# vsu/foo-dsp-bfir

Measured on AMD Instinct MI355X. Metric: Msamples/s (output channel-samples), 8ch 131072-tap FIR @4096-sample partitions, higher is better.
Workload: dtype f32; 1 GPU; cfg3_8ch_131072tap_L4096_fp32; channels=8, taps=131072, partition=4096, fft_size=8192, partitions=32, blocks_per_launch=4096, engines_rank0=1, channels_rank0=8, streams_total=1, io=interleaved frames resident in HBM (generated there), parallelism=one independent stream per rank, no collective

## Files before the change

foo-dsp-bfir_amd/csrc/fft_lds.h:

```cpp
#pragma once
#include <hip/hip_runtime.h>

#include <type_traits>

namespace bfir {

template <typename T, int P> __device__ __forceinline__ void pin_registers(T (&re)[P], T (&im)[P])
{
#pragma unroll
    for (int e = 0; e < P; e++) asm volatile("" : "+v"(re[e]), "+v"(im[e]));
}

template <typename T> struct Vec2;
template <> struct Vec2<float>  { using type = float2; };
template <> struct Vec2<double> { using type = double2; };
template <typename T> struct Vec4;
template <> struct Vec4<float>  { using type = float4; };
template <> struct Vec4<double> { using type = double4; };

template <int LOG2M> struct FftCfg;
#define BFIR_FFT_CFG(lg, nt, np, a, b, c, d)                                   \
    template <> struct FftCfg<lg> {                                            \
        static constexpr int NT = nt, NP = np, R0 = a, R1 = b, R2 = c, R3 = d; \
    };
BFIR_FFT_CFG(4, 4, 2, 4, 4, 1, 1)
BFIR_FFT_CFG(5, 4, 2, 8, 4, 1, 1)
BFIR_FFT_CFG(6, 8, 2, 8, 8, 1, 1)
BFIR_FFT_CFG(7, 16, 3, 8, 4, 4, 1)
BFIR_FFT_CFG(8, 16, 2, 16, 16, 1, 1)
BFIR_FFT_CFG(9, 32, 3, 16, 8, 4, 1)
BFIR_FFT_CFG(10, 64, 3, 16, 16, 4, 1)
BFIR_FFT_CFG(11, 128, 3, 16, 16, 8, 1)
BFIR_FFT_CFG(12, 256, 3, 16, 16, 16, 1)
BFIR_FFT_CFG(13, 512, 4, 16, 16, 8, 4)
BFIR_FFT_CFG(14, 1024, 4, 16, 16, 16, 4)
#undef BFIR_FFT_CFG

constexpr int BFIR_MIN_LOG2M = 4;
constexpr int BFIR_MAX_LOG2M = 14;

template <typename T>
__device__ __forceinline__ void cmul(T &re, T &im, T wr, T wi)
{
    T tr = re * wr - im * wi;
    T ti = re * wi + im * wr;
    re = tr; im = ti;
}

template <int MM, int SIGN, typename T>
__device__ __forceinline__ void mul_w16(T &re, T &im)
{
// ... 91 lines not shown

template <int LO, int HI, typename Fn> __device__ __forceinline__ void static_for(Fn &&f)
{
    if constexpr (LO < HI) {
        f(std::integral_constant<int, LO>{});
        static_for<LO + 1, HI>(f);
    }
}

__host__ __device__ constexpr int tw_nbase(int R) { return R == 16 ? 6 : R == 8 ? 4 : R == 4 ? 2 : 1; }
__host__ __device__ constexpr int tw_base_exp(int R, int j)
{
    return R == 16 ? (j < 4 ? j + 1 : 4 * (j - 2)) : j + 1;
}

template <typename T, int LOG2M, int SIGN> struct LdsFft {
    using Cfg = FftCfg<LOG2M>;
    using V2 = typename Vec2<T>::type;
    static constexpr int M = 1 << LOG2M;
    static constexpr int NT = Cfg::NT;
    static constexpr int P = M / NT;
    static constexpr int NP = Cfg::NP;

    __host__ __device__ static constexpr int radix(int s)
    {
        return s == 0 ? Cfg::R0 : s == 1 ? Cfg::R1 : s == 2 ? Cfg::R2 : Cfg::R3;
    }
    __host__ __device__ static constexpr int pprod(int s)
    {
        int p = 1;
        for (int j = 0; j < s; j++) p *= radix(j);
        return p;
    }
    __host__ __device__ static constexpr int twoff(int s)
    {
        int o = 0;
        for (int j = 1; j < s; j++) o += (radix(j) - 1) * pprod(j);
        return o;
    }
    __host__ __device__ static constexpr int twsize() { return twoff(NP); }

    static constexpr int LDS_ELEMS = M + M / 32;
    __host__ __device__ __forceinline__ static constexpr int phys(int i) { return i + (i >> 5); }

    __host__ __device__ __forceinline__ static constexpr int in_index(int tid, int e)
    {
        return (tid + (e / radix(0)) * NT) + (e % radix(0)) * (M / radix(0));
    }
    __host__ __device__ __forceinline__ static constexpr int out_index(int tid, int e)
    {
        return (tid + (e / radix(NP - 1)) * NT) + Dft<radix(NP - 1), SIGN, T>::inv(e % radix(NP - 1)) * (M / radix(NP - 1));
    }

    template <int S> static constexpr int ntw() { return S == 0 ? 1 : (P / radix(S)) * (radix(S) - 1); }

    template <int S>
    __device__ __forceinline__ static void load_twiddles(V2 (&w)[ntw<S>()], const V2 *__restrict__ tw, int tid)
    {
        constexpr int R = radix(S), p = pprod(S);
#pragma unroll
        for (int b = 0; b < P / R; b++) {
            const int k = (tid + b * NT) & (p - 1);
#pragma unroll
            for (int r = 1; r < R; r++) w[b * (R - 1) + r - 1] = tw[twoff(S) + (r - 1) * p + k];
        }
    }
// ... 25 lines not shown
        } else {
            exchange<S - 1>(re, im, lds, tid);
            load_twiddles<S>(w, tw, tid);
        }
        butterflies<S>(re, im, w);
    }

    template <int S> __host__ __device__ static constexpr int widx(int tid, int b, int q)
    {
        const int R = radix(S), p = pprod(S);
        const int i = tid + b * NT, k = i & (p - 1);
        return (i - k) * R + k + q * p;
    }
    template <int S> __host__ __device__ static constexpr int ridx(int tid, int b, int r)
    {
        return (tid + b * NT) + r * (M / radix(S + 1));
    }
    template <int S> __host__ __device__ static constexpr bool wr_affine()
    {
        for (int b = 0; b < P / radix(S); b++)
            for (int q = 0; q < radix(S); q++) {
                const int off = phys(widx<S>(0, b, q)) - phys(widx<S>(0, 0, 0));
                for (int t = 1; t < NT; t++)
                    if (phys(widx<S>(t, b, q)) - phys(widx<S>(t, 0, 0)) != off) return false;
            }
        return true;
    }
    template <int S> __host__ __device__ static constexpr bool rd_affine()
    {
        for (int b = 0; b < P / radix(S + 1); b++)
            for (int r = 0; r < radix(S + 1); r++) {
                const int off = phys(ridx<S>(0, b, r)) - phys(ridx<S>(0, 0, 0));
                for (int t = 1; t < NT; t++)
                    if (phys(ridx<S>(t, b, r)) - phys(ridx<S>(t, 0, 0)) != off) return false;
            }
        return true;
    }

    template <int S>
    __device__ __forceinline__ static void exchange(T *re, T *im, V2 *lds, int tid)
    {
        constexpr int R = radix(S), Rn = radix(S + 1);
        __syncthreads();
        if constexpr (wr_affine<S>()) {
            V2 *wp = lds + phys(widx<S>(tid, 0, 0));
            static_for<0, P / R>([&](auto B_) {
                constexpr int b = decltype(B_)::value;
                static_for<0, R>([&](auto Q_) {
                    constexpr int q = decltype(Q_)::value;
                    constexpr int off = phys(widx<S>(0, b, q)) - phys(widx<S>(0, 0, 0));
                    V2 v; v.x = re[b * R + Dft<R, SIGN, T>::pos(q)]; v.y = im[b * R + Dft<R, SIGN, T>::pos(q)];
                    wp[off] = v;
                });
            });
        } else {
#pragma unroll
            for (int b = 0; b < P / R; b++)
#pragma unroll
                for (int q = 0; q < R; q++) {
                    V2 v; v.x = re[b * R + Dft<R, SIGN, T>::pos(q)]; v.y = im[b * R + Dft<R, SIGN, T>::pos(q)];
                    lds[phys(widx<S>(tid, b, q))] = v;
                }
        }
        __syncthreads();
        if constexpr (rd_affine<S>()) {
            const V2 *rp = lds + phys(ridx<S>(tid, 0, 0));
            static_for<0, P / Rn>([&](auto B_) {
                constexpr int b = decltype(B_)::value;
                static_for<0, Rn>([&](auto R_) {
                    constexpr int r = decltype(R_)::value;
                    constexpr int off = phys(ridx<S>(0, b, r)) - phys(ridx<S>(0, 0, 0));
                    const V2 v = rp[off];
                    re[b * Rn + r] = v.x; im[b * Rn + r] = v.y;
                });
            });
        } else {
#pragma unroll
            for (int b = 0; b < P / Rn; b++)
#pragma unroll
                for (int r = 0; r < Rn; r++) {
                    V2 v = lds[phys(ridx<S>(tid, b, r))];
                    re[b * Rn + r] = v.x; im[b * Rn + r] = v.y;
                }
        }
#pragma unroll
        for (int e = 0; e < P; e++) asm volatile("" : "+v"(re[e]), "+v"(im[e]));
    }

    __host__ __device__ static constexpr int kspan(int s) { return pprod(s) < NT ? pprod(s) : NT; }
    __host__ __device__ static constexpr int boff(int s)
    {
        int o = 0;
        for (int j = 1; j < s; j++) o += tw_nbase(radix(j)) * kspan(j);
        return o;
    }
    __host__ __device__ static constexpr int bsize() { return boff(NP); }
    static constexpr int NBREG = NP > 1 ? tw_nbase(radix(NP - 1)) : 1;
    static constexpr int LDSB_ELEMS = NP > 2 ? boff(NP - 1) : 1;

    __device__ __forceinline__ static void load_bases(V2 (&B)[NBREG], V2 *ldsb, const V2 *__restrict__ twb, int tid)
    {
        if constexpr (NP > 2)
            for (int i = tid; i < LDSB_ELEMS; i += NT) ldsb[i] = twb[i];
        if constexpr (NP > 1)
            static_for<0, NBREG>([&](auto J_) {
                constexpr int J = decltype(J_)::value;
                B[J] = twb[boff(NP - 1) + J * kspan(NP - 1) + (tid & (kspan(NP - 1) - 1))];
            });
    }

    template <int S, int J> __device__ __forceinline__ static V2 base(const V2 (&B)[NBREG], const V2 *ldsb, int tid)
    {
        if constexpr (S == NP - 1) return B[J];
        else return ldsb[boff(S) + J * kspan(S) + (tid & (kspan(S) - 1))];
    }

    template <int S, int r> __device__ __forceinline__ static V2 base_twiddle(const V2 (&B)[NBREG], const V2 *ldsb, int tid)
    {
        constexpr int R = radix(S);
        if constexpr (R == 16 && (r & 3) != 0 && (r >> 2) != 0) {
            const V2 a = base<S, 2 + (r >> 2)>(B, ldsb, tid), c = base<S, (r & 3) - 1>(B, ldsb, tid);
            V2 w; w.x = a.x * c.x - a.y * c.y; w.y = a.x * c.y + a.y * c.x;
            return w;
        } else if constexpr (R == 16) {
            return base<S, ((r >> 2) == 0 ? r - 1 : 2 + (r >> 2))>(B, ldsb, tid);
        } else if constexpr (R == 8 && r > 4) {
            const V2 a = base<S, 3>(B, ldsb, tid), c = base<S, r - 5>(B, ldsb, tid);
            V2 w; w.x = a.x * c.x - a.y * c.y; w.y = a.x * c.y + a.y * c.x;
            return w;
        } else if constexpr (R == 4 && r == 3) {
            const V2 a = base<S, 0>(B, ldsb, tid), c = base<S, 1>(B, ldsb, tid);
            V2 w; w.x = a.x * c.x - a.y * c.y; w.y = a.x * c.y + a.y * c.x;
            return w;
        } else {
            return base<S, r - 1>(B, ldsb, tid);
        }
    }

    template <int S>
    __device__ __forceinline__ static void butterflies_tb(T *re, T *im, const V2 (&B)[NBREG], const V2 *ldsb, int tid)
    {
        constexpr int R = radix(S), p = pprod(S);
        static_assert(p <= NT || 16 * NT == p * R, "constant rotations are sixteenth roots of unity");
        static_for<1, R>([&](auto R_) {
            constexpr int r = decltype(R_)::value;
            if constexpr (R == 16 && (r & 3) == 0) __builtin_amdgcn_sched_barrier(0);
            const V2 w = base_twiddle<S, r>(B, ldsb, tid);
            static_for<0, P / R>([&](auto B_) {
                constexpr int b = decltype(B_)::value;
                constexpr int bp = b % (p > NT ? p / NT : 1);
                cmul(re[b * R + r], im[b * R + r], w.x, (T)(SIGN < 0 ? w.y : -w.y));
                if constexpr (bp != 0) mul_w16<(r * bp) % 16, SIGN>(re[b * R + r], im[b * R + r]);
            });
        });
        static_for<0, P / R>([&](auto B_) {
            constexpr int b = decltype(B_)::value;
            Dft<R, SIGN, T>::run(re + b * R, im + b * R);
        });
    }

    __device__ __forceinline__ static void run(T *re, T *im, V2 *lds, const V2 *__restrict__ tw, int tid)
    {
        {
            V2 w0[1];
            butterflies<0>(re, im, w0);
        }
        if constexpr (NP > 1) pass<1>(re, im, lds, tw, tid);
        if constexpr (NP > 2) pass<2>(re, im, lds, tw, tid);
        if constexpr (NP > 3) pass<3>(re, im, lds, tw, tid);
    }
};

}
```

foo-dsp-bfir_amd/csrc/kernels.hip:

```cpp
#include "kernels.h"

#include <algorithm>
#include <cmath>
#include <cstdio>
#include <cstdlib>
#include <vector>

#include "fft_lds.h"

namespace bfir {

constexpr int BFIR_MAXCH = 8;

#define BFIR_FOR_LOG2M(F) \
    F(4) F(5) F(6) F(7) F(8) F(9) F(10) F(11) F(12) F(13) F(14)

template <int LOG2M> static void fill_tw(std::vector<long double> &tw)
{
    using F = LdsFft<float, LOG2M, -1>;
    tw.assign(2 * (size_t)(F::twsize() > 0 ? F::twsize() : 1), 0.0L);
    const long double two_pi = 6.283185307179586476925286766559L;
    for (int s = 1; s < F::NP; s++) {
        const int R = F::radix(s), p = F::pprod(s);
        for (int r = 1; r < R; r++)
            for (int k = 0; k < p; k++) {
                long double ang = -two_pi * (long double)(r * k) / (long double)(p * R);
                size_t o = (size_t)F::twoff(s) + (size_t)(r - 1) * p + k;
                tw[2 * o] = cosl(ang);
                tw[2 * o + 1] = sinl(ang);
            }
    }
}

template <int LOG2M> static void fill_twb(std::vector<long double> &tw)
{
    using F = LdsFft<float, LOG2M, -1>;
    tw.assign(2 * (size_t)(F::bsize() > 0 ? F::bsize() : 1), 0.0L);
    const long double two_pi = 6.283185307179586476925286766559L;
    for (int s = 1; s < F::NP; s++) {
        const int R = F::radix(s), p = F::pprod(s), ks = F::kspan(s);
        for (int j = 0; j < tw_nbase(R); j++)
            for (int k0 = 0; k0 < ks; k0++) {
                long double ang = -two_pi * (long double)(tw_base_exp(R, j) * k0) / (long double)(p * R);
                size_t o = (size_t)F::boff(s) + (size_t)j * ks + k0;
                tw[2 * o] = cosl(ang);
                tw[2 * o + 1] = sinl(ang);
            }
    }
}

template <typename T> static void *upload(const std::vector<long double> &v)
{
    std::vector<T> h(v.size());
    for (size_t i = 0; i < v.size(); i++) h[i] = (T)v[i];
    void *d = nullptr;
    if (hipMalloc(&d, h.size() * sizeof(T)) != hipSuccess) return nullptr;
    if (hipMemcpy(d, h.data(), h.size() * sizeof(T), hipMemcpyHostToDevice) != hipSuccess) {
        (void)hipFree(d);
        return nullptr;
    }
    return d;
}

// ... 4 lines not shown
        BFIR_FOR_LOG2M(F)
#undef F
    }
    return 0;
}

int fft_plan_create(FftPlan *plan, int filter_length, int realsize)
{
    int lg = 0;
    while ((1 << lg) < filter_length) lg++;
    if ((1 << lg) != filter_length || lg < BFIR_MIN_LOG2M || lg > BFIR_MAX_LOG2M) return -1;
    if (realsize != 4 && realsize != 8) return -1;
    if (((size_t)filter_length + (size_t)filter_length / 32) * 2 * (size_t)realsize > 160 * 1024) return -1;
    std::vector<long double> tw, ws, twb;
    switch (lg) {
#define F(lgv) case lgv: fill_tw<lgv>(tw); fill_twb<lgv>(twb); break;
        BFIR_FOR_LOG2M(F)
#undef F
    }
    const int M = filter_length, N = 2 * M;
    ws.resize(2 * (size_t)M);
    const long double two_pi = 6.283185307179586476925286766559L;
    for (int k = 0; k < M; k++) {
        long double ang = -two_pi * (long double)k / (long double)N;
        ws[2 * k] = cosl(ang);
        ws[2 * k + 1] = sinl(ang);
    }
    plan->log2m = lg;
    plan->realsize = realsize;
    plan->tw = realsize == 4 ? upload<float>(tw) : upload<double>(tw);
    plan->ws = realsize == 4 ? upload<float>(ws) : upload<double>(ws);
// ... 2012 lines not shown
```

foo-dsp-bfir_amd/csrc/pair.hip:

```cpp
#include "kernels.h"

#include <algorithm>
#include <cstdlib>

#include "fft_lds.h"
#include "pair_io.h"

namespace bfir {

namespace {

template <int LOG2N>
__global__ __launch_bounds__(FftCfg<LOG2N>::NT, 4) void k_fwd_pair_ps(FwdPairArgs a, const float2 *__restrict__ twb, int run_len)
{
    using F = LdsFft<float, LOG2N, -1>;
    constexpr int N = F::M, NT = F::NT, P = F::P, L = N / 2, H = P / 2;
    static_assert(F::radix(0) == 16 && P == 16, "in_index(tid, e) = tid + e * (N / 16)");
    static_assert(F::phys(32) == 33 && F::phys(N - 1) == N - 1 + N / 32 - 1, "the split step's addresses assume i + (i >> 5)");
    __shared__ __attribute__((aligned(16))) float2 lds[F::LDS_ELEMS + 1];
    __shared__ __attribute__((aligned(16))) float2 ldsb[F::LDSB_ELEMS];

    const int tid = threadIdx.x;
    const int w = xcd_work_item(blockIdx.x, gridDim.x);
    const int half_c = a.C / 2, pairs = a.n_eng * half_c;
    const int rr = w / pairs, pp = w - rr * pairs;
    const float sc = 0.5f * a.scale;
    const int g = pp / half_c, cp = pp - g * half_c;
    const int C = a.C;
    const int t0 = rr * run_len, t1 = min(a.n_t, t0 + run_len);
    if (t0 >= t1) return;
// ... 48 lines not shown
            F::template butterflies<0>(re, im, w0);
        }
        static_for<1, F::NP>([&](auto S_) {
            constexpr int S = decltype(S_)::value;
            int tl = tid; asm volatile("" : "+v"(tl));
            F::template exchange<S - 1>(re, im, lds, tl);
            F::template butterflies_tb<S>(re, im, B, ldsb, tl);
            if constexpr (S == 1) {
                asm_prefetch8x2(nxt, fo, make_rsrc_words(raw + (long)(t + 1) * L * C, t + 1 < t1 ? blk_bytes : 0u), estep);
            }
        });

        int tz = tid; asm volatile("" : "+v"(tz));
        __syncthreads();
        {
            float2 *zw = lds + F::phys(tz);
            static_for<0, P>([&](auto E_) {
                constexpr int e = decltype(E_)::value;
                static_assert(F::out_index(0, e) % 32 == 0, "additive padding");
                float2 v; v.x = re[e]; v.y = im[e];
                zw[F::phys(F::out_index(0, e))] = v;
            });
        }
        __syncthreads();
        const long slot = (long)((a.base_slot + t) % a.ring) * N;
        const __amdgpu_buffer_rsrc_t rxa = make_rsrc(da0 + slot, (unsigned)N * 4u), rxb = make_rsrc(da0 + a.dst_ch_stride + slot, (unsigned)N * 4u);
        const float2 *zk = lds + F::phys(2 * tz);
        constexpr int OMAX = F::phys(2 * NT * (P / 4 - 1));
        const float2 *zn1 = lds + (F::phys(N - 1 - 2 * tz) - OMAX);
        const float2 *zn0 = zn1 + ((tz & 15) == 0 ? 2 : 1);
#pragma unroll
// ... 11 lines not shown
                const float2 zh = lds[F::phys(L)];
                const bool k0 = tz == 0;
                xa.x = k0 ? 2.f * zk0.x : xa.x; xa.y = k0 ? 2.f * zh.x : xa.y;
                xb.x = k0 ? 2.f * zk0.y : xb.x; xb.y = k0 ? 2.f * zh.y : xb.y;
            }
            buf_store4<2>(rxa, (unsigned)tz * 16u, (unsigned)(j * NT) * 16u, xa);
            buf_store4<2>(rxb, (unsigned)tz * 16u, (unsigned)(j * NT) * 16u, xb);
        }
    }
    asm_wait_vmcnt<0>(nxt);
}

template <int LOG2N>
__global__ __launch_bounds__(FftCfg<LOG2N>::NT, 4) void k_fwd_tp_ps(FwdPairArgs a, const float2 *__restrict__ twb, int run_len)
{
    using F = LdsFft<float, LOG2N, -1>;
    constexpr int N = F::M, NT = F::NT, P = F::P, L = N / 2, H = P / 2;
    static_assert(F::radix(0) == 16 && P == 16, "in_index(tid, e) = tid + e * (N / 16)");
    static_assert(F::phys(32) == 33 && F::phys(N - 1) == N - 1 + N / 32 - 1, "the split step's addresses assume i + (i >> 5)");
    __shared__ __attribute__((aligned(16))) float2 lds[F::LDS_ELEMS + 1];
    __shared__ __attribute__((aligned(16))) float2 ldsb[F::LDSB_ELEMS];

    const int tid = threadIdx.x;
    const int w = xcd_work_item(blockIdx.x, gridDim.x);
    const int C = a.C, units = a.n_eng * C;
    const int rr = w / units, pp = w - rr * units;
    const int g = pp / C, c = pp - g * C;
    const float sc = 0.5f * a.scale;
    const int t0 = rr * run_len, t1 = min(a.n_t, t0 + run_len);
    if (t0 >= t1) return;

// ... 57 lines not shown
        }
        static_for<1, F::NP>([&](auto S_) {
            constexpr int S = decltype(S_)::value;
            int tl = tid; asm volatile("" : "+v"(tl));
            F::template exchange<S - 1>(re, im, lds, tl);
            F::template butterflies_tb<S>(re, im, B, ldsb, tl);
            if constexpr (S == 1) {
                asm_prefetch2x8x1(nb, nc, fo, make_rsrc_words(raw + (long)(t + 2) * L * C, t + 2 < t1 ? blk_bytes : 0u),
                                  make_rsrc_words(raw + (long)(t + 3) * L * C, t + 3 < t1 ? blk_bytes : 0u), estep);
            }
        });

        int tz = tid; asm volatile("" : "+v"(tz));
        __syncthreads();
        {
            float2 *zw = lds + F::phys(tz);
            static_for<0, P>([&](auto E_) {
                constexpr int e = decltype(E_)::value;
                static_assert(F::out_index(0, e) % 32 == 0, "additive padding");
                float2 v; v.x = re[e]; v.y = im[e];
                zw[F::phys(F::out_index(0, e))] = v;
            });
        }
        __syncthreads();
        const long slot_a = (long)((a.base_slot + t) % a.ring) * N, slot_b = (long)((a.base_slot + t + 1) % a.ring) * N;
        const __amdgpu_buffer_rsrc_t rxa = make_rsrc(da0 + slot_a, (unsigned)N * 4u);
        const __amdgpu_buffer_rsrc_t rxb = make_rsrc(da0 + slot_b, t + 1 < a.n_t ? (unsigned)N * 4u : 0u);
        const float2 *zk = lds + F::phys(2 * tz);
        constexpr int OMAX = F::phys(2 * NT * (P / 4 - 1));
        const float2 *zn1 = lds + (F::phys(N - 1 - 2 * tz) - OMAX);
        const float2 *zn0 = zn1 + ((tz & 15) == 0 ? 2 : 1);
// ... 12 lines not shown
                const float2 zh = lds[F::phys(L)];
                const bool k0 = tz == 0;
                xa.x = k0 ? 2.f * zk0.x : xa.x; xa.y = k0 ? 2.f * zh.x : xa.y;
                xb.x = k0 ? 2.f * zk0.y : xb.x; xb.y = k0 ? 2.f * zh.y : xb.y;
            }
            buf_store4<2>(rxa, (unsigned)tz * 16u, (unsigned)(j * NT) * 16u, xa);
            buf_store4<2>(rxb, (unsigned)tz * 16u, (unsigned)(j * NT) * 16u, xb);
        }
    }
    asm_wait_vmcnt<0>(nb, nc);
}

template <int LOG2N>
__global__ __launch_bounds__(FftCfg<LOG2N>::NT, inv_ps_min_waves<LOG2N>()) void k_inv_pair_ps(InvPairArgs a, const float2 *__restrict__ twb, int run_len)
{
    using F = LdsFft<float, LOG2N, +1>;
    constexpr int N = F::M, NT = F::NT, P = F::P, L = N / 2, Q = P / 4;
    __shared__ __attribute__((aligned(16))) float2 lds[F::LDS_ELEMS];
    __shared__ __attribute__((aligned(16))) float2 ldsb[F::LDSB_ELEMS];
    __shared__ unsigned int red_max[NT / 64 > 0 ? NT / 64 : 1][2], red_cnt[NT / 64 > 0 ? NT / 64 : 1][2];

    const int tid = threadIdx.x;
    const int w = xcd_work_item(blockIdx.x, gridDim.x);
    const int half_c = a.C / 2, pairs = a.n_eng * half_c;
    const int rr = w / pairs, pp = w - rr * pairs;
    const int g = pp / half_c, cp = pp - g * half_c;
    const int C = a.C;
    const int FS = a.frame_stride ? a.frame_stride : C;
    const int gc = g * C + 2 * cp;
    const int t0 = rr * run_len, t1 = min(a.n_t, t0 + run_len);
    if (t0 >= t1) return;
// ... 56 lines not shown
        static_for<1, F::NP>([&](auto S_) {
            constexpr int S = decltype(S_)::value;
            int tl = tid; asm volatile("" : "+v"(tl));
            F::template exchange<S - 1>(re, im, lds, tl);
            F::template butterflies_tb<S>(re, im, B, ldsb, tl);
            if constexpr (S == 1) {
                const unsigned nbytes = t + 1 < t1 ? (unsigned)N * 4u : 0u;
                asm_prefetch2x4x4(qa, qb, (unsigned)tl * 16u, make_rsrc_words(ya0 + (long)(t + 1) * N, nbytes),
                                  make_rsrc_words(ya0 + a.y_ch_stride + (long)(t + 1) * N, nbytes), (unsigned)NT * 16u);
            }
        });

        const __amdgpu_buffer_rsrc_t ro = make_rsrc(out0 + (long)t * L * FS, blk_bytes);
        int to = tid; asm volatile("" : "+v"(to));
#pragma unroll
        for (int e = 0; e < P; e++) {
            const int n = F::out_index(to, e);
            if (F::out_index(0, e) < L) {
                float2 v; v.x = re[e]; v.y = im[e];
                buf_store2(ro, (unsigned)to * cio * 4u, (unsigned)F::out_index(0, e) * cio * 4u, v);
                c0 += (fabsf(v.x) > rmax) ? 1u : 0u;
                c1 += (fabsf(v.y) > rmax) ? 1u : 0u;
                pk0 = fmaxf(pk0, fabsf(v.x)); pk1 = fmaxf(pk1, fabsf(v.y));
                if (F::out_index(0, e) == 0) {
                    const bool nf = n == 0 && !(isfinite(v.x) && isfinite(v.y));
                    bad = (nf && t < bad) ? t : bad;
                }
            }
        }
    }
    asm_wait_vmcnt<0>(qa, qb);
    if (bad != 0x7fffffff) flag_bad(a, bad);
    unsigned int mx0 = __float_as_uint(pk0), mx1 = __float_as_uint(pk1);
#pragma unroll
    for (int o = 32; o > 0; o >>= 1) {
// ... 9 lines not shown
        DevOverflow *of = of_shard(a.overflow, a.of_shard_stride) + (gc + tid);
        if (n) atomicAdd(&of->n_overflows, n);
        if ((unsigned long long)m > *(volatile unsigned long long *)&of->largest_bits)
            atomicMax(&of->largest_bits, (unsigned long long)m);
    }
}

__device__ __forceinline__ void buf_store1(__amdgpu_buffer_rsrc_t r, unsigned voff, unsigned soff, float f)
{
    __builtin_amdgcn_raw_buffer_store_b32(__float_as_uint(f), r, voff, soff, 0);
}

template <int LOG2N>
__global__ __launch_bounds__(FftCfg<LOG2N>::NT, inv_ps_min_waves<LOG2N>()) void k_inv_tp_ps(InvPairArgs a, const float2 *__restrict__ twb, int run_len)
{
    using F = LdsFft<float, LOG2N, +1>;
    constexpr int N = F::M, NT = F::NT, P = F::P, L = N / 2, Q = P / 4;
    __shared__ __attribute__((aligned(16))) float2 lds[F::LDS_ELEMS];
    __shared__ __attribute__((aligned(16))) float2 ldsb[F::LDSB_ELEMS];
    __shared__ unsigned int red_max[NT / 64 > 0 ? NT / 64 : 1][2], red_cnt[NT / 64 > 0 ? NT / 64 : 1][2];

    const int tid = threadIdx.x;
    const int w = xcd_work_item(blockIdx.x, gridDim.x);
    const int C = a.C, units = a.n_eng * C;
    const int rr = w / units, pp = w - rr * units;
    const int g = pp / C, c = pp - g * C;
    const int gc = g * C + c;
    const int t0 = rr * run_len, t1 = min(a.n_t, t0 + run_len);
    if (t0 >= t1) return;

    float2 B[F::NBREG];
// ... 56 lines not shown
            int tl = tid; asm volatile("" : "+v"(tl));
            F::template exchange<S - 1>(re, im, lds, tl);
            F::template butterflies_tb<S>(re, im, B, ldsb, tl);
            if constexpr (S == 1) {
                asm_prefetch2x4x4(qa, qb, (unsigned)tl * 16u,
                                  make_rsrc_words(ya0 + (long)(t + 2) * N, t + 2 < t1 ? (unsigned)N * 4u : 0u),
                                  make_rsrc_words(ya0 + (long)(t + 3) * N, t + 3 < t1 ? (unsigned)N * 4u : 0u), (unsigned)NT * 16u);
            }
        });

        const bool has_b = t + 1 < a.n_t;
        const __amdgpu_buffer_rsrc_t roa = make_rsrc(out0 + (long)t * L * C, blk_bytes);
        const __amdgpu_buffer_rsrc_t rob = make_rsrc(out0 + (long)(t + 1) * L * C, has_b ? blk_bytes : 0u);
        int to = tid; asm volatile("" : "+v"(to));
#pragma unroll
        for (int e = 0; e < P; e++) {
            const int n = F::out_index(to, e);
            if (F::out_index(0, e) < L) {
                const float va = re[e], vb = has_b ? im[e] : 0.f;
                buf_store1(roa, (unsigned)to * cio * 4u, (unsigned)F::out_index(0, e) * cio * 4u, va);
                buf_store1(rob, (unsigned)to * cio * 4u, (unsigned)F::out_index(0, e) * cio * 4u, vb);
                c0 += (fabsf(va) > rmax) ? 1u : 0u;
                c1 += (fabsf(vb) > rmax) ? 1u : 0u;
                pk0 = fmaxf(pk0, fabsf(va)); pk1 = fmaxf(pk1, fabsf(vb));
                if (F::out_index(0, e) == 0) {
                    const bool na = n == 0 && !isfinite(va), nbb = n == 0 && has_b && !isfinite(vb);
                    bad = (na && t < bad) ? t : bad;
                    bad = (nbb && t + 1 < bad) ? t + 1 : bad;
                }
            }
        }
    }
    asm_wait_vmcnt<0>(qa, qb);
    if (bad != 0x7fffffff) flag_bad(a, bad);
    unsigned int mx0 = __float_as_uint(fmaxf(pk0, pk1)), mx1 = 0u;
    c0 += c1; c1 = 0u;
// ... 87 lines not shown
```

foo-dsp-bfir_amd/csrc/quad.hip:

```cpp
#include "kernels.h"

#include <algorithm>
#include <atomic>
#include <cstdint>
#include <cstdlib>

#include "fft_lds.h"
#include "pair_io.h"

namespace bfir {

namespace {

__device__ __forceinline__ void asm_prefetch2x4x4_out(u32x4 (&a)[4], u32x4 (&b)[4], unsigned voff, i32x4 ra, i32x4 rb, unsigned step)
{
    const unsigned s1 = __builtin_amdgcn_readfirstlane(step), s2 = 2 * s1, s3 = 3 * s1;
    asm volatile("s_nop 4\n\t"
                 "buffer_load_dwordx4 %0, %8, %9, 0 offen nt\n\t"
                 "buffer_load_dwordx4 %4, %8, %10, 0 offen nt\n\t"
                 "buffer_load_dwordx4 %1, %8, %9, %11 offen nt\n\t"
                 "buffer_load_dwordx4 %5, %8, %10, %11 offen nt\n\t"
                 "buffer_load_dwordx4 %2, %8, %9, %12 offen nt\n\t"
                 "buffer_load_dwordx4 %6, %8, %10, %12 offen nt\n\t"
                 "buffer_load_dwordx4 %3, %8, %9, %13 offen nt\n\t"
                 "buffer_load_dwordx4 %7, %8, %10, %13 offen nt"
                 : "=&v"(a[0]), "=&v"(a[1]), "=&v"(a[2]), "=&v"(a[3]), "=&v"(b[0]), "=&v"(b[1]), "=&v"(b[2]), "=&v"(b[3])
                 : "v"(voff), "s"(ra), "s"(rb), "s"(s1), "s"(s2), "s"(s3)
                 : "memory");
}

template <int LOG2N>
__global__ __launch_bounds__(FftCfg<LOG2N>::NT, inv_ps_min_waves<LOG2N>()) void k_inv_quad_ps(InvPairArgs a, const float2 *__restrict__ twb, int run_len)
{
    using F = LdsFft<float, LOG2N, +1>;
    constexpr int N = F::M, NT = F::NT, P = F::P, L = N / 2, Q = P / 4;
    constexpr int NW = NT / 64 > 0 ? NT / 64 : 1;
    __shared__ __attribute__((aligned(16))) float2 lds[F::LDS_ELEMS];
    __shared__ __attribute__((aligned(16))) float2 ldsb[F::LDSB_ELEMS];
    __shared__ unsigned int red_max[NW][4], red_cnt[NW][4];

    const int tid = threadIdx.x;
    const int w = xcd_work_item(blockIdx.x, gridDim.x);
    const int quarter_c = a.C / 4, units = a.n_eng * quarter_c;
    const int rr = w / units, pp = w - rr * units;
    const int g = pp / quarter_c, cq = pp - g * quarter_c;
    const int C = a.C;
    const int gc = g * C + 4 * cq;
    const int t0 = rr * run_len, t1 = min(a.n_t, t0 + run_len);
    if (t0 >= t1) return;
// ... 62 lines not shown
                int tl = tid; asm volatile("" : "+v"(tl));
                F::template exchange<S - 1>(re, im, lds, tl);
                F::template butterflies_tb<S>(re, im, B, ldsb, tl);
                if constexpr (S == 1) {
                    const int tn = t + PR;
                    const unsigned nbytes = tn < t1 ? (unsigned)N * 4u : 0u;
                    const float *yn = ya0 + (long)(2 - 2 * PR) * a.y_ch_stride + (long)tn * N;
                    asm_prefetch2x4x4_out(qa, qb, (unsigned)tl * 16u, make_rsrc_words(yn, nbytes),
                                          make_rsrc_words(yn + a.y_ch_stride, nbytes), (unsigned)NT * 16u);
                }
            });

            int to = tid; asm volatile("" : "+v"(to));
            u32x4 fo[P / 2];
#pragma unroll
            for (int e = 0; e < P; e++) {
                const int n = F::out_index(to, e);
                if (F::out_index(0, e) < L) {
                    float2 v; v.x = re[e]; v.y = im[e];
                    if constexpr (PR == 0) { hr[e] = v.x; hi[e] = v.y; }
                    else {
                        u32x4 &f = fo[F::out_index(0, e) / NT];
                        f.x = __float_as_uint(hr[e]); f.y = __float_as_uint(hi[e]); f.z = __float_as_uint(v.x); f.w = __float_as_uint(v.y);
                    }
                    cn[2 * PR] += (fabsf(v.x) > rmax) ? 1u : 0u;
                    cn[2 * PR + 1] += (fabsf(v.y) > rmax) ? 1u : 0u;
                    pk[2 * PR] = fmaxf(pk[2 * PR], fabsf(v.x)); pk[2 * PR + 1] = fmaxf(pk[2 * PR + 1], fabsf(v.y));
                    if (F::out_index(0, e) == 0) {
                        const bool nf = n == 0 && !(isfinite(v.x) && isfinite(v.y));
                        bad = (nf && t < bad) ? t : bad;
                    }
                }
            }
            if constexpr (PR == 1)
                asm_store8x4(fo, (unsigned)to * cio * 4u, make_rsrc_words(out0 + (long)t * L * C, blk_bytes), (unsigned)NT * cio * 4u);
        });
    }
    asm_wait_vmcnt<0>(qa, qb);
    if (bad != 0x7fffffff) flag_bad(a, bad);
    unsigned int mx[4];
#pragma unroll
    for (int c = 0; c < 4; c++) mx[c] = __float_as_uint(pk[c]);
#pragma unroll
    for (int o = 32; o > 0; o >>= 1) {
#pragma unroll
        for (int c = 0; c < 4; c++) {
            const unsigned int m = __shfl_xor(mx[c], o);
            mx[c] = m > mx[c] ? m : mx[c];
            cn[c] += __shfl_xor(cn[c], o);
        }
// ... 53 lines not shown
```

foo-dsp-bfir_amd/csrc/wide.hip:

```cpp
#include "kernels.h"

#include <algorithm>
#include <atomic>
#include <cstdint>
#include <cstdlib>

#include "fft_lds.h"
#include "pair_io.h"

namespace bfir {

namespace {

constexpr int WIDE_PF_PASS = 1;

__device__ __forceinline__ void asm_prefetch8x4_out(u32x4 (&d)[8], unsigned voff, i32x4 r, unsigned step)
{
    const unsigned s1 = __builtin_amdgcn_readfirstlane(step), s2 = 2 * s1, s3 = 3 * s1, s4 = 4 * s1, s5 = 5 * s1, s6 = 6 * s1, s7 = 7 * s1;
    asm volatile("s_nop 4\n\t"
                 "buffer_load_dwordx4 %0, %8, %9, 0 offen\n\t"
                 "buffer_load_dwordx4 %1, %8, %9, %10 offen\n\t"
                 "buffer_load_dwordx4 %2, %8, %9, %11 offen\n\t"
                 "buffer_load_dwordx4 %3, %8, %9, %12 offen\n\t"
                 "buffer_load_dwordx4 %4, %8, %9, %13 offen\n\t"
                 "buffer_load_dwordx4 %5, %8, %9, %14 offen\n\t"
                 "buffer_load_dwordx4 %6, %8, %9, %15 offen\n\t"
                 "buffer_load_dwordx4 %7, %8, %9, %16 offen"
                 : "=&v"(d[0]), "=&v"(d[1]), "=&v"(d[2]), "=&v"(d[3]), "=&v"(d[4]), "=&v"(d[5]), "=&v"(d[6]), "=&v"(d[7])
                 : "v"(voff), "s"(r), "s"(s1), "s"(s2), "s"(s3), "s"(s4), "s"(s5), "s"(s6), "s"(s7)
                 : "memory");
}

template <int LOG2N>
__global__ __launch_bounds__(FftCfg<LOG2N>::NT, 4) void k_fwd_wide_ps(FwdPairArgs a, const float2 *__restrict__ twb, int run_len)
{
    using F = LdsFft<float, LOG2N, -1>;
    constexpr int N = F::M, NT = F::NT, P = F::P, L = N / 2, H = P / 2;
    static_assert(F::radix(0) == 16 && P == 16, "in_index(tid, e) = tid + e * (N / 16)");
    static_assert(F::phys(32) == 33 && F::phys(N - 1) == N - 1 + N / 32 - 1, "the split step's addresses assume i + (i >> 5)");
    static_assert(WIDE_PF_PASS >= 1 && WIDE_PF_PASS < F::NP, "the prefetch goes under one of the passes behind the first");
    __shared__ __attribute__((aligned(16))) float2 lds[F::LDS_ELEMS + 1];
    __shared__ __attribute__((aligned(16))) float2 ldsb[F::LDSB_ELEMS];

    const int tid = threadIdx.x;
    const int w = xcd_work_item(blockIdx.x, gridDim.x);
    const int quarter_c = a.C / 4, units = a.n_eng * quarter_c;
    const int rr = w / units, pp = w - rr * units;
    const float sc = 0.5f * a.scale;
    const int g = pp / quarter_c, cq = pp - g * quarter_c;
    const int C = a.C;
    const int t0 = rr * run_len, t1 = min(a.n_t, t0 + run_len);
// ... 59 lines not shown
                F::template butterflies<0>(re, im, w0);
            }
            static_for<1, F::NP>([&](auto S_) {
                constexpr int S = decltype(S_)::value;
                int tl = tid; asm volatile("" : "+v"(tl));
                F::template exchange<S - 1>(re, im, lds, tl);
                F::template butterflies_tb<S>(re, im, B, ldsb, tl);
                if constexpr (PR == 1 && S == WIDE_PF_PASS) {
                    asm_prefetch8x4_out(nxt, fo, make_rsrc_words(raw + (long)(t + 1) * L * C, t + 1 < t1 ? blk_bytes : 0u), estep);
                }
            });

            int tz = tid; asm volatile("" : "+v"(tz));
            __syncthreads();
            {
                float2 *zw = lds + F::phys(tz);
                static_for<0, P>([&](auto E_) {
                    constexpr int e = decltype(E_)::value;
                    static_assert(F::out_index(0, e) % 32 == 0, "additive padding");
                    float2 v; v.x = re[e]; v.y = im[e];
                    zw[F::phys(F::out_index(0, e))] = v;
                });
            }
            __syncthreads();
            const long slot = (long)((a.base_slot + t) % a.ring) * N;
            float *da = da0 + (long)(2 * PR) * a.dst_ch_stride + slot;
            const __amdgpu_buffer_rsrc_t rxa = make_rsrc(da, (unsigned)N * 4u), rxb = make_rsrc(da + a.dst_ch_stride, (unsigned)N * 4u);
            const float2 *zk = lds + F::phys(2 * tz);
            constexpr int OMAX = F::phys(2 * NT * (P / 4 - 1));
            const float2 *zn1 = lds + (F::phys(N - 1 - 2 * tz) - OMAX);
            const float2 *zn0 = zn1 + ((tz & 15) == 0 ? 2 : 1);
// ... 65 lines not shown
```

Baseline: 115,500 Msamples/s.

## Cut fp32 8192-point FFT into three radix-16 passes plus lane-pair radix-2 via DPP

For the 8192-point fp32 partitioned FFT, the four-pass 16/16/8/4 decomposition is replaced by three radix-16 passes. The leftover factor of two is folded into the last pass as a radix-2 exchange between adjacent lanes using DPP fmac, so one LDS exchange round and its barriers are removed. Twiddle bases, LDS padding for the penultimate exchange, output indexing and the store addresses in the forward and inverse kernels are all adapted to the new lane-pair point ownership. The cost is extra twiddle multiplies and more LDS-resident bases in the last pass, plus a more intricate indexing scheme.

```diff
diff --git a/foo-dsp-bfir_amd/csrc/fft_lds.h b/foo-dsp-bfir_amd/csrc/fft_lds.h
--- a/foo-dsp-bfir_amd/csrc/fft_lds.h
+++ b/foo-dsp-bfir_amd/csrc/fft_lds.h
@@ -35,6 +35,11 @@
 BFIR_FFT_CFG(13, 512, 4, 16, 16, 8, 4)
 BFIR_FFT_CFG(14, 1024, 4, 16, 16, 16, 4)
 #undef BFIR_FFT_CFG
+
+template <int LOG2M> struct FftCfgPair32;
+template <> struct FftCfgPair32<13> {
+    static constexpr int NT = 512, NP = 3, R0 = 16, R1 = 16, R2 = 16, R3 = 1;
+};
 
 constexpr int BFIR_MIN_LOG2M = 4;
 constexpr int BFIR_MAX_LOG2M = 14;
@@ -156,8 +161,9 @@
     return R == 16 ? (j < 4 ? j + 1 : 4 * (j - 2)) : j + 1;
 }
 
-template <typename T, int LOG2M, int SIGN> struct LdsFft {
-    using Cfg = FftCfg<LOG2M>;
+template <typename T, int LOG2M, int SIGN, bool PAIR32 = false> struct LdsFft {
+    using Cfg = typename std::conditional<PAIR32, FftCfgPair32<LOG2M>, FftCfg<LOG2M>>::type;
+    static_assert(!PAIR32 || std::is_same<T, float>::value, "the lane-pair cut is an fp32 one");
     using V2 = typename Vec2<T>::type;
     static constexpr int M = 1 << LOG2M;
     static constexpr int NT = Cfg::NT;
@@ -182,8 +188,13 @@
     }
     __host__ __device__ static constexpr int twsize() { return twoff(NP); }
 
-    static constexpr int LDS_ELEMS = M + M / 32;
+    static constexpr int XPAD = PAIR32 ? 16 : 0;
+    static constexpr int LDS_ELEMS = M + M / 32 + XPAD;
     __host__ __device__ __forceinline__ static constexpr int phys(int i) { return i + (i >> 5); }
+    template <int S> __host__ __device__ __forceinline__ static constexpr int xphys(int i)
+    {
+        return phys(i) + ((PAIR32 && S == NP - 2 && i >= M / 2) ? XPAD : 0);
+    }
 
     __host__ __device__ __forceinline__ static constexpr int in_index(int tid, int e)
     {
@@ -191,7 +202,21 @@
     }
     __host__ __device__ __forceinline__ static constexpr int out_index(int tid, int e)
     {
-        return (tid + (e / radix(NP - 1)) * NT) + Dft<radix(NP - 1), SIGN, T>::inv(e % radix(NP - 1)) * (M / radix(NP - 1));
+        if constexpr (PAIR32)
+            return (tid >> 1) + (M / 32) * (tid & 1) + Dft<16, SIGN, T>::inv(e) * (M / 16);
+        else
+            return (tid + (e / radix(NP - 1)) * NT) + Dft<radix(NP - 1), SIGN, T>::inv(e % radix(NP - 1)) * (M / radix(NP - 1));
+    }
+    template <bool OUT> __host__ __device__ static constexpr bool index_is_bijection()
+    {
+        bool seen[M] = {};
+        for (int t = 0; t < NT; t++)
+            for (int e = 0; e < P; e++) {
+                const int i = OUT ? out_index(t, e) : in_index(t, e);
+                if (i < 0 || i >= M || seen[i]) return false;
+                seen[i] = true;
+            }
+        return true;
     }
 
     template <int S> static constexpr int ntw() { return S == 0 ? 1 : (P / radix(S)) * (radix(S) - 1); }
@@ -247,15 +272,18 @@
     }
     template <int S> __host__ __device__ static constexpr int ridx(int tid, int b, int r)
     {
-        return (tid + b * NT) + r * (M / radix(S + 1));
+        if constexpr (PAIR32 && S + 1 == NP - 1)
+            return (tid >> 1) + (M / 2) * (tid & 1) + r * (M / 32);
+        else
+            return (tid + b * NT) + r * (M / radix(S + 1));
     }
     template <int S> __host__ __device__ static constexpr bool wr_affine()
     {
         for (int b = 0; b < P / radix(S); b++)
             for (int q = 0; q < radix(S); q++) {
-                const int off = phys(widx<S>(0, b, q)) - phys(widx<S>(0, 0, 0));
+                const int off = xphys<S>(widx<S>(0, b, q)) - xphys<S>(widx<S>(0, 0, 0));
                 for (int t = 1; t < NT; t++)
-                    if (phys(widx<S>(t, b, q)) - phys(widx<S>(t, 0, 0)) != off) return false;
+                    if (xphys<S>(widx<S>(t, b, q)) - xphys<S>(widx<S>(t, 0, 0)) != off) return false;
             }
         return true;
     }
@@ -263,9 +291,9 @@
     {
         for (int b = 0; b < P / radix(S + 1); b++)
             for (int r = 0; r < radix(S + 1); r++) {
-                const int off = phys(ridx<S>(0, b, r)) - phys(ridx<S>(0, 0, 0));
+                const int off = xphys<S>(ridx<S>(0, b, r)) - xphys<S>(ridx<S>(0, 0, 0));
                 for (int t = 1; t < NT; t++)
-                    if (phys(ridx<S>(t, b, r)) - phys(ridx<S>(t, 0, 0)) != off) return false;
+                    if (xphys<S>(ridx<S>(t, b, r)) - xphys<S>(ridx<S>(t, 0, 0)) != off) return false;
             }
         return true;
     }
@@ -276,12 +304,12 @@
         constexpr int R = radix(S), Rn = radix(S + 1);
         __syncthreads();
         if constexpr (wr_affine<S>()) {
-            V2 *wp = lds + phys(widx<S>(tid, 0, 0));
+            V2 *wp = lds + xphys<S>(widx<S>(tid, 0, 0));
             static_for<0, P / R>([&](auto B_) {
                 constexpr int b = decltype(B_)::value;
                 static_for<0, R>([&](auto Q_) {
                     constexpr int q = decltype(Q_)::value;
-                    constexpr int off = phys(widx<S>(0, b, q)) - phys(widx<S>(0, 0, 0));
+                    constexpr int off = xphys<S>(widx<S>(0, b, q)) - xphys<S>(widx<S>(0, 0, 0));
                     V2 v; v.x = re[b * R + Dft<R, SIGN, T>::pos(q)]; v.y = im[b * R + Dft<R, SIGN, T>::pos(q)];
                     wp[off] = v;
                 });
@@ -292,17 +320,17 @@
 #pragma unroll
                 for (int q = 0; q < R; q++) {
                     V2 v; v.x = re[b * R + Dft<R, SIGN, T>::pos(q)]; v.y = im[b * R + Dft<R, SIGN, T>::pos(q)];
-                    lds[phys(widx<S>(tid, b, q))] = v;
+                    lds[xphys<S>(widx<S>(tid, b, q))] = v;
                 }
         }
         __syncthreads();
         if constexpr (rd_affine<S>()) {
-            const V2 *rp = lds + phys(ridx<S>(tid, 0, 0));
+            const V2 *rp = lds + xphys<S>(ridx<S>(tid, 0, 0));
             static_for<0, P / Rn>([&](auto B_) {
                 constexpr int b = decltype(B_)::value;
                 static_for<0, Rn>([&](auto R_) {
                     constexpr int r = decltype(R_)::value;
-                    constexpr int off = phys(ridx<S>(0, b, r)) - phys(ridx<S>(0, 0, 0));
+                    constexpr int off = xphys<S>(ridx<S>(0, b, r)) - xphys<S>(ridx<S>(0, 0, 0));
                     const V2 v = rp[off];
                     re[b * Rn + r] = v.x; im[b * Rn + r] = v.y;
                 });
@@ -312,7 +340,7 @@
             for (int b = 0; b < P / Rn; b++)
 #pragma unroll
                 for (int r = 0; r < Rn; r++) {
-                    V2 v = lds[phys(ridx<S>(tid, b, r))];
+                    V2 v = lds[xphys<S>(ridx<S>(tid, b, r))];
                     re[b * Rn + r] = v.x; im[b * Rn + r] = v.y;
                 }
         }
@@ -320,31 +348,41 @@
         for (int e = 0; e < P; e++) asm volatile("" : "+v"(re[e]), "+v"(im[e]));
     }
 
-    __host__ __device__ static constexpr int kspan(int s) { return pprod(s) < NT ? pprod(s) : NT; }
+    __host__ __device__ static constexpr bool paired(int s) { return PAIR32 && s == NP - 1; }
+    __host__ __device__ static constexpr int kspan(int s) { return paired(s) ? NT : pprod(s) < NT ? pprod(s) : NT; }
+    __host__ __device__ static constexpr int nbase(int s) { return paired(s) ? 7 : tw_nbase(radix(s)); }
+    __host__ __device__ static constexpr int base_den(int s) { return paired(s) ? M : pprod(s) * radix(s); }
+    __host__ __device__ static constexpr int base_num(int s, int j, int k0)
+    {
+        if (!paired(s)) return tw_base_exp(radix(s), j) * k0;
+        return j < 6 ? tw_base_exp(16, j) * ((k0 >> 1) + (M / 32) * (k0 & 1)) : (k0 & 1) * (M / 2 + 16 * (k0 >> 1));
+    }
     __host__ __device__ static constexpr int boff(int s)
     {
         int o = 0;
-        for (int j = 1; j < s; j++) o += tw_nbase(radix(j)) * kspan(j);
+        for (int j = 1; j < s; j++) o += nbase(j) * kspan(j);
         return o;
     }
     __host__ __device__ static constexpr int bsize() { return boff(NP); }
-    static constexpr int NBREG = NP > 1 ? tw_nbase(radix(NP - 1)) : 1;
-    static constexpr int LDSB_ELEMS = NP > 2 ? boff(NP - 1) : 1;
+    static constexpr int NBLDS = PAIR32 ? 3 : 0;
+    static constexpr int NBREG = NP > 1 ? nbase(NP - 1) - NBLDS : 1;
+    static constexpr int LDSB_ELEMS = NP > 2 ? boff(NP - 1) + NBLDS * kspan(NP - 1) : 1;
 
     __device__ __forceinline__ static void load_bases(V2 (&B)[NBREG], V2 *ldsb, const V2 *__restrict__ twb, int tid)
     {
+        static_assert(!PAIR32 || (index_is_bijection<false>() && index_is_bijection<true>()), "every point in one (thread, slot)");
         if constexpr (NP > 2)
             for (int i = tid; i < LDSB_ELEMS; i += NT) ldsb[i] = twb[i];
         if constexpr (NP > 1)
             static_for<0, NBREG>([&](auto J_) {
                 constexpr int J = decltype(J_)::value;
-                B[J] = twb[boff(NP - 1) + J * kspan(NP - 1) + (tid & (kspan(NP - 1) - 1))];
+                B[J] = twb[boff(NP - 1) + (NBLDS + J) * kspan(NP - 1) + (tid & (kspan(NP - 1) - 1))];
             });
     }
 
     template <int S, int J> __device__ __forceinline__ static V2 base(const V2 (&B)[NBREG], const V2 *ldsb, int tid)
     {
-        if constexpr (S == NP - 1) return B[J];
+        if constexpr (S == NP - 1 && J >= NBLDS) return B[J - NBLDS];
         else return ldsb[boff(S) + J * kspan(S) + (tid & (kspan(S) - 1))];
     }
 
@@ -370,11 +408,53 @@
         }
     }
 
+    __device__ __forceinline__ static void paired_radix2(T *re, T *im, V2 f, int tid)
+    {
+        static_assert(std::is_same<T, float>::value, "32-bit DPP");
+        const T fy = SIGN < 0 ? f.y : -f.y;
+        const T s = __uint_as_float(0xbf800000u ^ ((unsigned)tid << 31));
+#pragma unroll
+        for (int e = 0; e < P; e++) cmul(re[e], im[e], f.x, fy);
+        __builtin_amdgcn_sched_barrier(0);
+        static_assert(P % 4 == 0, "groups of four points");
+#pragma unroll
+        for (int e = 0; e < P; e += 4)
+            asm volatile("s_nop 1\n\t"
+                         "v_fmac_f32_dpp %0, %0, %8 quad_perm:[1,0,3,2] row_mask:0xf bank_mask:0xf\n\t"
+                         "v_fmac_f32_dpp %1, %1, %8 quad_perm:[1,0,3,2] row_mask:0xf bank_mask:0xf\n\t"
+                         "v_fmac_f32_dpp %2, %2, %8 quad_perm:[1,0,3,2] row_mask:0xf bank_mask:0xf\n\t"
+                         "v_fmac_f32_dpp %3, %3, %8 quad_perm:[1,0,3,2] row_mask:0xf bank_mask:0xf\n\t"
+                         "v_fmac_f32_dpp %4, %4, %8 quad_perm:[1,0,3,2] row_mask:0xf bank_mask:0xf\n\t"
+                         "v_fmac_f32_dpp %5, %5, %8 quad_perm:[1,0,3,2] row_mask:0xf bank_mask:0xf\n\t"
+                         "v_fmac_f32_dpp %6, %6, %8 quad_perm:[1,0,3,2] row_mask:0xf bank_mask:0xf\n\t"
+                         "v_fmac_f32_dpp %7, %7, %8 quad_perm:[1,0,3,2] row_mask:0xf bank_mask:0xf"
+                         : "+v"(re[e]), "+v"(im[e]), "+v"(re[e + 1]), "+v"(im[e + 1]), "+v"(re[e + 2]), "+v"(im[e + 2]),
+                           "+v"(re[e + 3]), "+v"(im[e + 3])
+                         : "v"(s));
+    }
+
     template <int S>
     __device__ __forceinline__ static void butterflies_tb(T *re, T *im, const V2 (&B)[NBREG], const V2 *ldsb, int tid)
     {
         constexpr int R = radix(S), p = pprod(S);
         static_assert(p <= NT || 16 * NT == p * R, "constant rotations are sixteenth roots of unity");
+        if constexpr (paired(S)) {
+            paired_radix2(re, im, base<S, 6>(B, ldsb, tid), tid);
+            static_for<0, 4>([&](auto C_) {
+                constexpr int c = decltype(C_)::value;
+                __builtin_amdgcn_sched_barrier(0);
+                static_for<0, 4>([&](auto A_) {
+                    constexpr int r = 4 * decltype(A_)::value + c;
+                    if constexpr (r != 0) {
+                        const V2 w = base_twiddle<S, r>(B, ldsb, tid);
+                        cmul(re[r], im[r], w.x, (T)(SIGN < 0 ? w.y : -w.y));
+                    }
+                });
+            });
+            __builtin_amdgcn_sched_barrier(0);
+            Dft<R, SIGN, T>::run(re, im);
+            return;
+        }
         static_for<1, R>([&](auto R_) {
             constexpr int r = decltype(R_)::value;
             if constexpr (R == 16 && (r & 3) == 0) __builtin_amdgcn_sched_barrier(0);
@@ -394,6 +474,7 @@
 
     __device__ __forceinline__ static void run(T *re, T *im, V2 *lds, const V2 *__restrict__ tw, int tid)
     {
+        static_assert(!PAIR32, "the table-twiddle path keeps the per-size cut");
         {
             V2 w0[1];
             butterflies<0>(re, im, w0);
@@ -404,4 +485,7 @@
     }
 };
 
-}
+template <int LOG2M> constexpr bool ps_pair32() { return LOG2M == 13; }
+template <int LOG2M, int SIGN> using PsFft = LdsFft<float, LOG2M, SIGN, ps_pair32<LOG2M>()>;
+
+}
diff --git a/foo-dsp-bfir_amd/csrc/kernels.hip b/foo-dsp-bfir_amd/csrc/kernels.hip
--- a/foo-dsp-bfir_amd/csrc/kernels.hip
+++ b/foo-dsp-bfir_amd/csrc/kernels.hip
@@ -32,21 +32,26 @@
     }
 }
 
-template <int LOG2M> static void fill_twb(std::vector<long double> &tw)
-{
-    using F = LdsFft<float, LOG2M, -1>;
+template <typename F> static void fill_twb_of(std::vector<long double> &tw)
+{
     tw.assign(2 * (size_t)(F::bsize() > 0 ? F::bsize() : 1), 0.0L);
     const long double two_pi = 6.283185307179586476925286766559L;
     for (int s = 1; s < F::NP; s++) {
-        const int R = F::radix(s), p = F::pprod(s), ks = F::kspan(s);
-        for (int j = 0; j < tw_nbase(R); j++)
+        const int ks = F::kspan(s);
+        for (int j = 0; j < F::nbase(s); j++)
             for (int k0 = 0; k0 < ks; k0++) {
-                long double ang = -two_pi * (long double)(tw_base_exp(R, j) * k0) / (long double)(p * R);
+                long double ang = -two_pi * (long double)F::base_num(s, j, k0) / (long double)F::base_den(s);
                 size_t o = (size_t)F::boff(s) + (size_t)j * ks + k0;
                 tw[2 * o] = cosl(ang);
                 tw[2 * o + 1] = sinl(ang);
             }
     }
+}
+
+template <int LOG2M> static void fill_twb(std::vector<long double> &tw, int realsize)
+{
+    if (realsize == 4) fill_twb_of<PsFft<LOG2M, -1>>(tw);
+    else fill_twb_of<LdsFft<double, LOG2M, -1>>(tw);
 }
 
 template <typename T> static void *upload(const std::vector<long double> &v)
@@ -81,7 +86,7 @@
     if (((size_t)filter_length + (size_t)filter_length / 32) * 2 * (size_t)realsize > 160 * 1024) return -1;
     std::vector<long double> tw, ws, twb;
     switch (lg) {
-#define F(lgv) case lgv: fill_tw<lgv>(tw); fill_twb<lgv>(twb); break;
+#define F(lgv) case lgv: fill_tw<lgv>(tw); fill_twb<lgv>(twb, realsize); break;
         BFIR_FOR_LOG2M(F)
 #undef F
     }
diff --git a/foo-dsp-bfir_amd/csrc/pair.hip b/foo-dsp-bfir_amd/csrc/pair.hip
--- a/foo-dsp-bfir_amd/csrc/pair.hip
+++ b/foo-dsp-bfir_amd/csrc/pair.hip
@@ -13,7 +13,7 @@
 template <int LOG2N>
 __global__ __launch_bounds__(FftCfg<LOG2N>::NT, 4) void k_fwd_pair_ps(FwdPairArgs a, const float2 *__restrict__ twb, int run_len)
 {
-    using F = LdsFft<float, LOG2N, -1>;
+    using F = PsFft<LOG2N, -1>;
     constexpr int N = F::M, NT = F::NT, P = F::P, L = N / 2, H = P / 2;
     static_assert(F::radix(0) == 16 && P == 16, "in_index(tid, e) = tid + e * (N / 16)");
     static_assert(F::phys(32) == 33 && F::phys(N - 1) == N - 1 + N / 32 - 1, "the split step's addresses assume i + (i >> 5)");
@@ -92,7 +92,7 @@
         int tz = tid; asm volatile("" : "+v"(tz));
         __syncthreads();
         {
-            float2 *zw = lds + F::phys(tz);
+            float2 *zw = lds + F::phys(F::out_index(tz, 0));
             static_for<0, P>([&](auto E_) {
                 constexpr int e = decltype(E_)::value;
                 static_assert(F::out_index(0, e) % 32 == 0, "additive padding");
@@ -134,7 +134,7 @@
 template <int LOG2N>
 __global__ __launch_bounds__(FftCfg<LOG2N>::NT, 4) void k_fwd_tp_ps(FwdPairArgs a, const float2 *__restrict__ twb, int run_len)
 {
-    using F = LdsFft<float, LOG2N, -1>;
+    using F = PsFft<LOG2N, -1>;
     constexpr int N = F::M, NT = F::NT, P = F::P, L = N / 2, H = P / 2;
     static_assert(F::radix(0) == 16 && P == 16, "in_index(tid, e) = tid + e * (N / 16)");
     static_assert(F::phys(32) == 33 && F::phys(N - 1) == N - 1 + N / 32 - 1, "the split step's addresses assume i + (i >> 5)");
@@ -222,7 +222,7 @@
         int tz = tid; asm volatile("" : "+v"(tz));
         __syncthreads();
         {
-            float2 *zw = lds + F::phys(tz);
+            float2 *zw = lds + F::phys(F::out_index(tz, 0));
             static_for<0, P>([&](auto E_) {
                 constexpr int e = decltype(E_)::value;
                 static_assert(F::out_index(0, e) % 32 == 0, "additive padding");
@@ -265,7 +265,7 @@
 template <int LOG2N>
 __global__ __launch_bounds__(FftCfg<LOG2N>::NT, inv_ps_min_waves<LOG2N>()) void k_inv_pair_ps(InvPairArgs a, const float2 *__restrict__ twb, int run_len)
 {
-    using F = LdsFft<float, LOG2N, +1>;
+    using F = PsFft<LOG2N, +1>;
     constexpr int N = F::M, NT = F::NT, P = F::P, L = N / 2, Q = P / 4;
     __shared__ __attribute__((aligned(16))) float2 lds[F::LDS_ELEMS];
     __shared__ __attribute__((aligned(16))) float2 ldsb[F::LDSB_ELEMS];
@@ -352,11 +352,14 @@
         const __amdgpu_buffer_rsrc_t ro = make_rsrc(out0 + (long)t * L * FS, blk_bytes);
         int to = tid; asm volatile("" : "+v"(to));
 #pragma unroll
+        for (int e = 0; e < P; e++)
+            if (F::out_index(0, e) < L) asm volatile("" : "+v"(re[e]), "+v"(im[e]));
+#pragma unroll
         for (int e = 0; e < P; e++) {
             const int n = F::out_index(to, e);
             if (F::out_index(0, e) < L) {
                 float2 v; v.x = re[e]; v.y = im[e];
-                buf_store2(ro, (unsigned)to * cio * 4u, (unsigned)F::out_index(0, e) * cio * 4u, v);
+                buf_store2(ro, (unsigned)F::out_index(to, 0) * cio * 4u, (unsigned)F::out_index(0, e) * cio * 4u, v);
                 c0 += (fabsf(v.x) > rmax) ? 1u : 0u;
                 c1 += (fabsf(v.y) > rmax) ? 1u : 0u;
                 pk0 = fmaxf(pk0, fabsf(v.x)); pk1 = fmaxf(pk1, fabsf(v.y));
@@ -396,7 +399,7 @@
 template <int LOG2N>
 __global__ __launch_bounds__(FftCfg<LOG2N>::NT, inv_ps_min_waves<LOG2N>()) void k_inv_tp_ps(InvPairArgs a, const float2 *__restrict__ twb, int run_len)
 {
-    using F = LdsFft<float, LOG2N, +1>;
+    using F = PsFft<LOG2N, +1>;
     constexpr int N = F::M, NT = F::NT, P = F::P, L = N / 2, Q = P / 4;
     __shared__ __attribute__((aligned(16))) float2 lds[F::LDS_ELEMS];
     __shared__ __attribute__((aligned(16))) float2 ldsb[F::LDSB_ELEMS];
@@ -483,12 +486,15 @@
         const __amdgpu_buffer_rsrc_t rob = make_rsrc(out0 + (long)(t + 1) * L * C, has_b ? blk_bytes : 0u);
         int to = tid; asm volatile("" : "+v"(to));
 #pragma unroll
+        for (int e = 0; e < P; e++)
+            if (F::out_index(0, e) < L) asm volatile("" : "+v"(re[e]), "+v"(im[e]));
+#pragma unroll
         for (int e = 0; e < P; e++) {
             const int n = F::out_index(to, e);
             if (F::out_index(0, e) < L) {
                 const float va = re[e], vb = has_b ? im[e] : 0.f;
-                buf_store1(roa, (unsigned)to * cio * 4u, (unsigned)F::out_index(0, e) * cio * 4u, va);
-                buf_store1(rob, (unsigned)to * cio * 4u, (unsigned)F::out_index(0, e) * cio * 4u, vb);
+                buf_store1(roa, (unsigned)F::out_index(to, 0) * cio * 4u, (unsigned)F::out_index(0, e) * cio * 4u, va);
+                buf_store1(rob, (unsigned)F::out_index(to, 0) * cio * 4u, (unsigned)F::out_index(0, e) * cio * 4u, vb);
                 c0 += (fabsf(va) > rmax) ? 1u : 0u;
                 c1 += (fabsf(vb) > rmax) ? 1u : 0u;
                 pk0 = fmaxf(pk0, fabsf(va)); pk1 = fmaxf(pk1, fabsf(vb));
diff --git a/foo-dsp-bfir_amd/csrc/quad.hip b/foo-dsp-bfir_amd/csrc/quad.hip
--- a/foo-dsp-bfir_amd/csrc/quad.hip
+++ b/foo-dsp-bfir_amd/csrc/quad.hip
@@ -32,7 +32,7 @@
 template <int LOG2N>
 __global__ __launch_bounds__(FftCfg<LOG2N>::NT, inv_ps_min_waves<LOG2N>()) void k_inv_quad_ps(InvPairArgs a, const float2 *__restrict__ twb, int run_len)
 {
-    using F = LdsFft<float, LOG2N, +1>;
+    using F = PsFft<LOG2N, +1>;
     constexpr int N = F::M, NT = F::NT, P = F::P, L = N / 2, Q = P / 4;
     constexpr int NW = NT / 64 > 0 ? NT / 64 : 1;
     __shared__ __attribute__((aligned(16))) float2 lds[F::LDS_ELEMS];
@@ -125,6 +125,9 @@
             int to = tid; asm volatile("" : "+v"(to));
             u32x4 fo[P / 2];
 #pragma unroll
+            for (int e = 0; e < P; e++)
+                if (F::out_index(0, e) < L) asm volatile("" : "+v"(re[e]), "+v"(im[e]));
+#pragma unroll
             for (int e = 0; e < P; e++) {
                 const int n = F::out_index(to, e);
                 if (F::out_index(0, e) < L) {
@@ -144,7 +147,7 @@
                 }
             }
             if constexpr (PR == 1)
-                asm_store8x4(fo, (unsigned)to * cio * 4u, make_rsrc_words(out0 + (long)t * L * C, blk_bytes), (unsigned)NT * cio * 4u);
+                asm_store8x4(fo, (unsigned)F::out_index(to, 0) * cio * 4u, make_rsrc_words(out0 + (long)t * L * C, blk_bytes), (unsigned)NT * cio * 4u);
         });
     }
     asm_wait_vmcnt<0>(qa, qb);
diff --git a/foo-dsp-bfir_amd/csrc/wide.hip b/foo-dsp-bfir_amd/csrc/wide.hip
--- a/foo-dsp-bfir_amd/csrc/wide.hip
+++ b/foo-dsp-bfir_amd/csrc/wide.hip
@@ -34,7 +34,7 @@
 template <int LOG2N>
 __global__ __launch_bounds__(FftCfg<LOG2N>::NT, 4) void k_fwd_wide_ps(FwdPairArgs a, const float2 *__restrict__ twb, int run_len)
 {
-    using F = LdsFft<float, LOG2N, -1>;
+    using F = PsFft<LOG2N, -1>;
     constexpr int N = F::M, NT = F::NT, P = F::P, L = N / 2, H = P / 2;
     static_assert(F::radix(0) == 16 && P == 16, "in_index(tid, e) = tid + e * (N / 16)");
     static_assert(F::phys(32) == 33 && F::phys(N - 1) == N - 1 + N / 32 - 1, "the split step's addresses assume i + (i >> 5)");
@@ -124,7 +124,7 @@
             int tz = tid; asm volatile("" : "+v"(tz));
             __syncthreads();
             {
-                float2 *zw = lds + F::phys(tz);
+                float2 *zw = lds + F::phys(F::out_index(tz, 0));
                 static_for<0, P>([&](auto E_) {
                     constexpr int e = decltype(E_)::value;
                     static_assert(F::out_index(0, e) % 32 == 0, "additive padding");
```

After: 116,500 Msamples/s (median of 6 runs). Within noise of the previous version (+0.8%).
